# ypw0102/GDR

Measured on AMD Instinct MI355X. Metric: queries/sec on NQ-320k (768-d), higher is better.
Workload: dtype f32; 1 GPU; C2/ragged/prefilter: t5-base encoder 512 q/GPU + Q.D^T top-100, 320000x768 corpus; batch_per_gpu=512, global_batch=512, seq_len=40, corpus_rows=320000, dim=768, k=100, encoder_rows=ragged

## Files before the change

### gdr_amd/_ffi.py

```python
import ctypes as C
import os

_HERE = os.path.dirname(os.path.abspath(__file__))
LIB_PATH = os.environ.get("GDR_HIP_LIB") or os.path.join(_HERE, "libgdr_hip.so")

GDR_OK, GDR_EINVAL, GDR_ENOSPC, GDR_EHIP = 0, -1, -2, -3
ABI_VERSION = 9
RERANK_POSITIONS = 1
RERANK_CHUNKED = 2
SIM_EXHAUSTIVE = 1
SIM_NO_STREAM = 2
EPI_NONE, EPI_RESIDUAL, EPI_RELU, EPI_BIAS, EPI_BIAS_RELU, EPI_BIAS_RESIDUAL, EPI_BIAS_GELU = range(7)
(F32_FORM_TILES, F32_FORM_PERSISTENT, F32_FORM_SMALL, F32_FORM_SMALL_SPLITK, F32_FORM_SPLITK, F32_FORM_STREAMK_256,
 F32_FORM_STREAMK_TAIL) = range(1, 8)
STREAMK_WS_BYTES = 33558528


class GdrError(RuntimeError):
    pass


class GdrT5Dims(C.Structure):
    _fields_ = [("vocab_size", C.c_int32), ("d_model", C.c_int32), ("d_kv", C.c_int32), ("d_ff", C.c_int32),
                ("num_heads", C.c_int32), ("num_layers", C.c_int32), ("rel_buckets", C.c_int32),
# ... 57 lines not shown
SIGNATURES = {
    "gdr_last_error": (C.c_char_p, []),
    "gdr_abi_version": (_i, []),
    "gdr_device_fault_pending": (_i, []),
    "gdr_device_fault_clear": (None, []),
    "gdr_device_fault_inject_for_tests": (None, []),
    "gdr_prof_enable": (_i, [_i]),
    "gdr_prof_collect": (_i, [C.POINTER(C.c_int64), C.POINTER(C.c_double), C.POINTER(C.c_double)]),
    "gdr_linear_f32": (_i, [_vp, _i64, _vp, _i64, _vp, _i64, _i64, _i, _i, _i, _vp, _vp, _i64, _vp]),
    "gdr_linear_bf16": (_i, [_vp, _i64, _vp, _i64, _vp, _i64, _i64, _i, _i, _i, _vp, _vp, _i64, _vp]),
    "gdr_split_row_elems": (_i, [_i, _i]),
    "gdr_split_f32_f16x2": (_i, [_vp, _vp, _i64, _i, _i64, _vp]),
    "gdr_split_f32_bf16x3": (_i, [_vp, _vp, _i64, _i, _i64, _vp]),
    "gdr_linear_split_bf16": (_i, [_vp, _i64, _vp, _i64, _vp, _i64, _i64, _i, _i, _i, _i, _vp, _vp, _i64, _vp]),
    "gdr_linear_bf16_tile_form": (_i, [_i64, _i, _i, _i]),
    "gdr_linear_f32_form": (_i, [_i64, _i, _i, _sz]),
    "gdr_linear_f32_splitk": (_i, [_vp, _i64, _vp, _i64, _vp, _i64, _i64, _i, _i, _i, _vp, _vp, _i64, _vp, _sz, _vp]),
    "gdr_l2_normalize": (_i, [_vp, _vp, _i64, _i, _f, _vp]),
    "gdr_t5_layer_norm": (_i, [_vp, _vp, _vp, _i64, _i, _f, _vp]),
    "gdr_t5_encoder_workspace_bytes": (_sz, [C.POINTER(GdrT5Dims), _i, _i]),
    "gdr_t5_encoder_forward": (_i, [C.POINTER(GdrT5EncoderWeights), _vp, _vp, _i, _i, _vp, _vp, _vp, _sz, _vp]),
    "gdr_t5_encoder_ragged_workspace_bytes": (_sz, [C.POINTER(GdrT5Dims), _i, _i]),
    "gdr_t5_encoder_forward_ragged": (_i, [C.POINTER(GdrT5EncoderWeights), _vp, _vp, _i, _i, _vp, _vp, _i64, _vp, _sz, _vp]),
    "gdr_t5_encoder_forward_ragged_bf16": (_i, [C.POINTER(GdrT5EncoderWeights), _vp, _vp, _i, _i, _vp, _vp, _i64, _vp, _sz, _vp]),
    "gdr_t5_encoder_split_workspace_bytes": (_sz, [C.POINTER(GdrT5Dims), _i, _i]),
    "gdr_t5_encoder_forward_ragged_split": (_i, [C.POINTER(GdrT5EncoderWeights), _vp, _vp, _i, _i, _vp, _vp, _i64, _i, _vp, _sz, _vp]),
    "gdr_t5_encoder_bf16_workspace_bytes": (_sz, [C.POINTER(GdrT5Dims), _i, _i]),
    "gdr_t5_encoder_forward_bf16": (_i, [C.POINTER(GdrT5EncoderWeights), _vp, _vp, _i, _i, _vp, _vp, _vp, _sz, _vp]),
    "gdr_sim_topk_workspace_bytes": (_sz, [_i, _i64, _i, _i, _i]),
    "gdr_sim_topk": (_i, [_vp, _i, _vp, _i64, _i, _i, C.c_int32, _vp, _vp, _vp, _i, _vp, _sz, _vp]),
# ... 104 lines not shown
```

### gdr_amd/csrc/encoder.hip

```cpp
#include <stdlib.h>

#include "layers.h"

namespace gdr {

constexpr size_t ENC_SPLITK_BYTES = (size_t)112 << 20;
static_assert(STREAMK_BYTES <= ENC_SPLITK_BYTES, "stream-K scratch must fit the split-K region");
constexpr bool ENC_LAST_Q_CLS_DEFAULT = true;

static int enc_streamk(char* splitk_region, StreamK* sk, hipStream_t stream) {
  sk->part = reinterpret_cast<float*>(splitk_region);
  sk->flag = reinterpret_cast<int32_t*>(splitk_region + STREAMK_PART_BYTES);
  sk->epoch = 0;
  if (hipMemsetAsync(sk->flag, 0, 512 * sizeof(int32_t), stream) != hipSuccess) {
    set_error("t5_encoder: memset of the stream-K flags failed");
    return GDR_EHIP;
  }
  return GDR_OK;
}

struct EncWs {
  size_t off_h, off_nx, off_qkv, off_ctx, off_ff, off_splitk, off_bf, total;
};

// ... 297 lines not shown
  at.ldq = at.ldk = at.ldv = 3 * inner, at.ldo = inner;
  at.q_bstride = at.k_bstride = at.o_bstride = L;
  at.B = B, at.H = H, at.dk = dk, at.Lq = L, at.Lk = L;
  at.q_pos0 = 0, at.scale = 1.0f;
  at.rel_bias = w->rel_bias, at.bidirectional = 1, at.num_buckets = dm.rel_buckets;
  at.lut = make_bucket_lut(dm.rel_buckets / 2, dm.rel_max_distance);
  at.key_mask = mask, at.mask_bstride = L, at.causal = 0, at.causal_neg_inf = 0;
  at.kv_rows = nullptr, at.kv_group = 1;
  at.seq_off = seq_off, at.seq_len = seq_len;

  const bool pooled_only = out_hidden == nullptr && big;
  static const bool last_q_cls_on = [] {
    const char* e = getenv("GDR_ENC_LAST_Q_CLS");
    return e ? atoi(e) != 0 : ENC_LAST_Q_CLS_DEFAULT;
  }();
  for (int i = 0; i < dm.num_layers; ++i) {
    const GdrT5EncLayer& ly = w->layers[i];
    GDR_CHECK_ARG(ly.ln_attn && ly.wqkv && ly.wo && ly.ln_ff && ly.wi && ly.wo_ff, "t5_encoder_ragged: layer %d null weight", i);
    if (i == 0 && qkv0) {
    } else if (pooled_only && i == dm.num_layers - 1 && last_q_cls_on) {
      if ((rc = launch_rmsnorm_dev(h, ly.ln_attn, nx, rows_dev, M, d, dm.eps, stream))) return rc;
      if ((rc = linear(nx, d, ly.wqkv + (size_t)inner * d, qkv + inner, 3 * inner, 2 * inner, d, GDR_EPI_NONE, nullptr))) return rc;
      if ((rc = launch_gather_rows(nx, seq_off, B, d, nx_cls, stream))) return rc;
      if ((rc = launch_linear_f32(nx_cls, d, ly.wqkv, d, ctx_cls, inner, B, inner, d, GDR_EPI_NONE, nullptr, nullptr, 0, stream)))
        return rc;
      if ((rc = launch_scatter_rows_strided(ctx_cls, seq_off, B, inner, qkv, 3 * inner, stream))) return rc;
    } else {
      if ((rc = launch_rmsnorm_dev(h, ly.ln_attn, nx, rows_dev, M, d, dm.eps, stream))) return rc;
      if ((rc = linear(nx, d, ly.wqkv, qkv, 3 * inner, 3 * inner, d, GDR_EPI_NONE, nullptr))) return rc;
    }
    if ((rc = launch_attention(at, stream))) return rc;
    if (pooled_only && i == dm.num_layers - 1) {
      if ((rc = launch_gather_rows(ctx, seq_off, B, inner, ctx_cls, stream))) return rc;
      if ((rc = launch_gather_rows(h, seq_off, B, d, h_cls, stream))) return rc;
      if ((rc = launch_linear_f32(ctx_cls, inner, ly.wo, inner, h_cls, d, B, d, inner, GDR_EPI_RESIDUAL, nullptr, h_cls, d, stream)))
        return rc;
      if ((rc = launch_rmsnorm(h_cls, ly.ln_ff, nx_cls, B, d, dm.eps, nullptr, 1, stream))) return rc;
      if ((rc = launch_linear_f32(nx_cls, d, ly.wi, d, ff_cls, dm.d_ff, B, dm.d_ff, d, GDR_EPI_RELU, nullptr, nullptr, 0, stream)))
        return rc;
      if ((rc = launch_linear_f32(ff_cls, dm.d_ff, ly.wo_ff, dm.d_ff, h_cls, d, B, d, dm.d_ff, GDR_EPI_RESIDUAL, nullptr, h_cls, d,
                                  stream)))
        return rc;
      return launch_rmsnorm(h_cls, w->final_ln, out_pooled, B, d, dm.eps, nullptr, 1, stream);
    }
    if ((rc = linear(ctx, inner, ly.wo, h, d, d, inner, GDR_EPI_RESIDUAL, h))) return rc;
// ... 193 lines not shown
```

### gdr_amd/csrc/gemm_bf16.hip

```cpp
#include "common.h"

namespace gdr {

typedef float f32x4b __attribute__((ext_vector_type(4)));
typedef __bf16 bf16x8b __attribute__((ext_vector_type(8)));
typedef _Float16 f16x8b __attribute__((ext_vector_type(8)));

struct Bf16GemmArgs {
  const char* A;
  const char* W;
  float* C;
  const float* bias;
  const float* residual;
  int64_t lda, ldw, ldc, ldr;
  int64_t M;
  int64_t Nrows;
  int N, K, tiles_n;
  int has_bias, has_residual, act;
  int out_bf16;
  const int64_t* m_dev;
  int split_k0;
  const float* dot_h;
  int64_t dot_ldh;
  const int32_t* dot_rows;
  const float* dot_e;
  float* dot_out;
  float dot_scale;
  int dot_d;
  SimEpilogue sim;
};

__device__ __forceinline__ float gelu_erf_b(float x) { return 0.5f * x * (1.0f + erff(x * 0.70710678118654752440f)); }

template <int SPLIT>
__device__ __forceinline__ int plane_of(int p, bool is_w) {
  if (SPLIT == 1) return ((is_w ? 0x102010 : 0x120100) >> (4 * p)) & 3;
  return ((is_w ? 0x001 : 0x010) >> (4 * p)) & 3;
}
template <int SPLIT>
__device__ __forceinline__ void ktile_offsets(int kt, int p, int k0, int split_k0, int& off_a, int& off_w) {
  if (SPLIT == 0) {
    off_a = off_w = kt * 128;
    return;
  }
// ... 305 lines not shown
            g.C[m * g.ldc + n + j] = x;
        }
      }
    }
  }
}

#pragma clang diagnostic push
#pragma clang diagnostic ignored "-Winline-asm"
#define GLDS16(gptr_, lds_) \
  asm volatile("s_mov_b32 m0, %0\n\ts_nop 0\n\tglobal_load_lds_dwordx4 %1, off" ::"s"(lds_), "v"(gptr_) : "memory", "m0")

constexpr int HALF_BYTES = 128 * 128;
constexpr int OFF_A_LO = 0, OFF_A_HI = HALF_BYTES, OFF_B_LO = 2 * HALF_BYTES, OFF_B_HI = 3 * HALF_BYTES, BUF_BYTES = 4 * HALF_BYTES;

template <int BN, int SPLIT = 0>
__global__ __launch_bounds__(512, 1) void gemm_nt_bf16_tile256_kernel(const Bf16GemmArgs g) {
  static_assert(BN == 256 || BN == 192, "tile width");
  constexpr int WCOLS = BN / 4;
  constexpr int NBH = BN == 256 ? 2 : 1;
  constexpr int NB = 2 + NBH;
  constexpr int HI_ROWS = 16 * NBH;
  extern __shared__ __attribute__((aligned(1024))) char smem256[];
  unsigned bid = blockIdx.x;
  const int64_t Mv = g.m_dev ? *g.m_dev : g.M;
  const int tiles_n = (g.N + BN - 1) / BN;
  {
    unsigned nblk = gridDim.x;
    if (g.m_dev) {
      const int64_t live = ((Mv + 255) / 256) * (int64_t)tiles_n;
      if (live < (int64_t)nblk) {
        if ((int64_t)bid >= live) return;
        nblk = (unsigned)live;
      }
    }
    const unsigned q_ = nblk >> 3, r_ = nblk & 7u, xcd_ = bid & 7u, j_ = bid >> 3;
    bid = (xcd_ < r_ ? xcd_ * (q_ + 1) : r_ * (q_ + 1) + (xcd_ - r_) * q_) + j_;
  }
  const int64_t m0 = (int64_t)(bid / (unsigned)tiles_n) * 256;
  if (m0 >= Mv) return;
  const int n0 = (int)(bid % (unsigned)tiles_n) * BN;
  const int tid = threadIdx.x, wave = tid >> 6, lane = tid & 63;
  const int wr = wave >> 2, wc = wave & 3, r16 = lane & 15, q4 = lane >> 4;
  const unsigned lds0 = __builtin_amdgcn_readfirstlane((unsigned)(uintptr_t)(__attribute__((address_space(3))) char*)(smem256));
  const int srow = lane >> 3, schunk = lane & 7;
  const char* a_src[2][2];
  const char* b_lo_src[2];
  const char* b_hi_src[NBH];
#pragma unroll
  for (int h = 0; h < 2; ++h)
#pragma unroll
    for (int i = 0; i < 2; ++i) {
      const int lr = (wave * 2 + i) * 8 + srow;
      const int chunk = schunk ^ ((lr >> 1) & 7);
      int64_t ra = m0 + (lr >> 6) * 128 + h * 64 + (lr & 63);
      ra = ra < Mv ? ra : Mv - 1;
      a_src[h][i] = g.A + (ra * g.lda) * 2 + chunk * 16;
    }
#pragma unroll
  for (int i = 0; i < 2; ++i) {
    const int lr = (wave * 2 + i) * 8 + srow;
    const int chunk = schunk ^ ((lr >> 1) & 7);
    int rb = n0 + (lr >> 5) * WCOLS + (lr & 31);
    rb = rb < g.N ? rb : g.N - 1;
    b_lo_src[i] = g.W + ((int64_t)rb * g.ldw) * 2 + chunk * 16;
  }
#pragma unroll
  for (int i = 0; i < NBH; ++i) {
    const int lr = NBH == 2 ? (wave * 2 + i) * 8 + srow : wave * 8 + srow;
    const int chunk = schunk ^ ((lr >> 1) & 7);
    int rb = n0 + (lr / HI_ROWS) * WCOLS + 32 + (lr % HI_ROWS);
    rb = rb < g.N ? rb : g.N - 1;
    b_hi_src[i] = g.W + ((int64_t)rb * g.ldw) * 2 + chunk * 16;
  }
  const unsigned st_dst = lds0 + (unsigned)__builtin_amdgcn_readfirstlane(wave) * 2048;
  const unsigned st_dst1 = lds0 + (unsigned)__builtin_amdgcn_readfirstlane(wave) * 1024;
#define STAGE(src_, half_off_, buf_, koff_)                                                 \
  {                                                                                         \
    GLDS16(src_[0] + (koff_), st_dst + (buf_)*BUF_BYTES + (half_off_));                     \
    GLDS16(src_[1] + (koff_), st_dst + (buf_)*BUF_BYTES + (half_off_) + 1024);              \
  }
#define STAGE_BHI(buf_, koff_)                                                              \
  {                                                                                         \
    if (NBH == 2) STAGE(b_hi_src, OFF_B_HI, buf_, koff_)                                    \
    else GLDS16(b_hi_src[0] + (koff_), st_dst1 + (buf_)*BUF_BYTES + OFF_B_HI);              \
  }
  const int sw = (r16 >> 1) & 7;
  const int c0 = (q4 ^ sw) << 4;
// ... 127 lines not shown
    STAGE(a_src[0], OFF_A_LO, 1, a_o3)
    BAR()
    asm volatile("s_waitcnt lgkmcnt(0)" ::: "memory");
    __builtin_amdgcn_sched_barrier(0);
    MFMA_Q(1, 2, NBH, fbh)
    BAR()
    STAGE_BHI(1, w_o3)
    WAIT_3HALVES()
    BAR()
    MFMA_Q(1, 0, 2, fbl)
    BAR()
    a_o1 = a_o3;
  }
  asm volatile("s_waitcnt vmcnt(0)" ::: "memory");
  if (wr == 0) BAR()
#pragma unroll
  for (int mi = 0; mi < 8; ++mi) {
    const int64_t m = m0 + wr * 128 + mi * 16 + r16;
    if (m >= Mv) continue;
#pragma unroll
    for (int ni = 0; ni < NB; ++ni) {
      const int n = n0 + wc * WCOLS + ni * 16 + 4 * q4;
      if (n >= g.N) continue;
      float v[4] = {acc[mi][ni][0], acc[mi][ni][1], acc[mi][ni][2], acc[mi][ni][3]};
      if (g.has_bias) {
        const float4 b = *reinterpret_cast<const float4*>(g.bias + n);
        v[0] += b.x, v[1] += b.y, v[2] += b.z, v[3] += b.w;
      }
      if (g.has_residual) {
        const float4 r = *reinterpret_cast<const float4*>(g.residual + m * g.ldr + n);
// ... 136 lines not shown
  g.lda = lda, g.ldw = ldw, g.M = M, g.N = N, g.Nrows = N, g.K = K;
  g.tiles_n = N / 128;
  g.m_dev = m_dev;
  g.dot_h = h, g.dot_ldh = ldh, g.dot_rows = rows_map, g.dot_e = E, g.dot_out = partial, g.dot_scale = scale, g.dot_d = dot_d;
  int64_t blocks = ((M + 127) / 128) * g.tiles_n;
  if (blocks <= 0) return 0;
  if (blocks > 0x7fffffffLL) {
    set_error("linear_bf16(head dot): grid too large");
    return GDR_EINVAL;
  }
  hipLaunchKernelGGL((gemm_nt_bf16_glds_kernel<3, 128>), dim3((unsigned)blocks), dim3(256), 0, stream, g);
  GDR_CHECK_LAUNCH("gemm_nt_bf16_glds_kernel(head dot)");
  return 0;
}

int launch_sim_bf16_glds(const void* D, int64_t N, const void* Q, int B, int d, const SimEpilogue& ep, int64_t n_doc_tiles,
                         hipStream_t stream) {
  if (d % 64 != 0 || ((uintptr_t)D & 15) || ((uintptr_t)Q & 15)) return 1;
  Bf16GemmArgs g{};
  g.A = static_cast<const char*>(Q), g.W = static_cast<const char*>(D);
  g.lda = d, g.ldw = d, g.M = B, g.Nrows = N, g.N = 0, g.K = d;
  g.tiles_n = (B + 127) / 128;
  g.sim = ep;
  const int64_t blocks = n_doc_tiles * g.tiles_n;
  if (blocks <= 0) return 0;
  if (blocks > 0x7fffffffLL) {
    set_error("sim_bf16: grid too large");
    return GDR_EINVAL;
  }
  if (ep.mode == 1)
    hipLaunchKernelGGL(gemm_nt_bf16_glds_kernel<1>, dim3((unsigned)blocks), dim3(256), 0, stream, g);
  else
    hipLaunchKernelGGL(gemm_nt_bf16_glds_kernel<2>, dim3((unsigned)blocks), dim3(256), 0, stream, g);
  GDR_CHECK_LAUNCH("gemm_nt_bf16_glds_kernel(sim)");
  return 0;
}

}

extern "C" int gdr_linear_bf16_tile_form(int64_t M, int N, int K, int epilogue) {
  const int has_residual = epilogue == GDR_EPI_RESIDUAL || epilogue == GDR_EPI_BIAS_RESIDUAL;
  return gdr::linear_bf16_tile_form(M, N, K, has_residual, 0);
}

namespace gdr {
__global__ __launch_bounds__(256) void split_f32_bf16x3_kernel(const float* __restrict__ in, int64_t ld_in, __bf16* __restrict__ out,
                                                              int64_t ld_out, int64_t rows, int K, const int64_t* __restrict__ rows_dev,
                                                              int form) {
  const int k4 = K >> 2;
  const int64_t i = (int64_t)blockIdx.x * 256 + threadIdx.x;
  const int64_t r = i / k4;
  const int c = (int)(i - r * k4) * 4;
  if (r >= (rows_dev ? *rows_dev : rows)) return;
// ... 53 lines not shown
```

### gdr_amd/csrc/gemm_small.hip

```cpp
#include <stdlib.h>

#include "common.h"

namespace gdr {

typedef float f32x16m __attribute__((ext_vector_type(16)));

constexpr int SB = 64, SBK = 32, SLD = SBK + 4;

struct SmallGemmArgs {
  const float* A;
  const float* W;
  float* C;
  const float* bias;
  const float* residual;
  int64_t lda, ldw, ldc, ldr;
  int64_t M;
  int N, K, tiles_n, tiles_m;
  int has_bias, has_residual, act;
  int ksplit, kchunk;
  const int64_t* m_dev;
  const int32_t* live;
};

// ... 97 lines not shown
#undef S_STORE
#undef S_COMPUTE
  if (g.ksplit > 1) {
    float* slab = g.C + ((int64_t)tile * g.ksplit + split) * (SB * SB);
#pragma unroll
    for (int r = 0; r < 16; ++r) slab[(wm * 32 + (r & 3) + 8 * (r >> 2) + 4 * h) * SB + wn * 32 + l31] = acc[r];
    return;
  }
  const int n = n0 + wn * 32 + l31;
  if (n >= g.N) return;
  const float bia = g.has_bias ? g.bias[n] : 0.f;
#pragma unroll
  for (int r = 0; r < 16; ++r) {
    const int64_t m = m0 + wm * 32 + (r & 3) + 8 * (r >> 2) + 4 * h;
    if (m >= Mrows) continue;
    float v = acc[r] + bia;
    if (g.has_residual) v += g.residual[m * g.ldr + n];
    if (g.act == 1) v = fmaxf(v, 0.f);
    if (g.act == 2) v = gelu_erf_s(v);
    g.C[m * g.ldc + n] = v;
  }
}

__global__ __launch_bounds__(256) void splitk_reduce_small_kernel(const float* __restrict__ partial, int S, int tiles_n,
                                                                  int64_t M, int N, float* __restrict__ C, int64_t ldc,
                                                                  const float* __restrict__ bias,
                                                                  const float* __restrict__ residual, int64_t ldr,
                                                                  int act, const int64_t* __restrict__ m_dev,
                                                                  const int32_t* __restrict__ live) {
  if (live && *live == 0) return;
// ... 139 lines not shown
  SmallGemmArgs g{};
  g.A = A, g.W = W, g.bias = bias, g.residual = residual;
  g.lda = lda, g.ldw = ldw, g.ldc = ldc, g.ldr = ldr, g.M = M, g.N = N, g.K = K, g.tiles_n = tiles_n;
  g.ksplit = S, g.kchunk = chunk_steps * SBK;
  g.m_dev = m_dev, g.live = live;
  g.tiles_m = (int)tiles_m;
  const double flops = 2.0 * (double)M * (double)N * (double)K;
  if (ne && (S == 1 || N % 4 != 0 || N > 1024 || act > 1)) return 2;
  if (slabs) {
    if (has_bias || has_residual || act || ne) return 1;
    slabs->part = nullptr, slabs->S = 1, slabs->tiles_n = tiles_n;
  }
  if (S == 1) {
    g.C = C, g.has_bias = has_bias, g.has_residual = has_residual, g.act = act;
    ProfScope prof(PROF_LINEAR, flops, stream);
    hipLaunchKernelGGL(gemm_nt_f32_small_kernel, dim3((unsigned)tiles), dim3(256), 0, stream, g);
    GDR_CHECK_LAUNCH("gemm_nt_f32_small_kernel");
    return 0;
  }
  g.C = ws;
  {
    ProfScope prof(PROF_LINEAR, flops, stream);
    hipLaunchKernelGGL(gemm_nt_f32_small_kernel, dim3((unsigned)(tiles * S)), dim3(256), 0, stream, g);
  }
  GDR_CHECK_LAUNCH("gemm_nt_f32_small_kernel(split)");
  if (slabs) {
    slabs->part = ws, slabs->S = S, slabs->tiles_n = tiles_n;
    return 0;
  }
  ProfScope prof_r(PROF_REDUCE, 0.0, stream);
// ... 16 lines not shown
```

### gdr_amd/csrc/layers.h

```cpp
#pragma once
#include "common.h"

namespace gdr {

struct BucketLut {
  uint8_t v[128];
};
BucketLut make_bucket_lut(int nb, int max_distance);

struct AttnArgs {
  const float* q;
  const float* k;
  const float* v;
  float* out;
  void* out_bf16;
  int64_t ldq, ldk, ldv, ldo;
  int64_t q_bstride, k_bstride, o_bstride;
  int B, H, dk, Lq, Lk;
  int q_pos0;
  float scale;
  const float* rel_bias;
  int bidirectional, num_buckets;
  BucketLut lut;
  const int64_t* key_mask;
  int64_t mask_bstride;
  int causal;
  int causal_neg_inf;
  const int32_t* kv_rows;
  int kv_group;
  int q_same_pos;
  const int32_t* seq_off;
  const int32_t* seq_len;
  int qkv_bf16;
  const int64_t* b_count_dev;
  const float* q_part;
  int q_S, q_tiles_n;
  const int32_t* live;
};
int launch_attention(const AttnArgs& a, hipStream_t stream);
int launch_attention_long(const AttnArgs& a, hipStream_t stream);

int launch_embed(const float* table, const int64_t* ids, int64_t rows, int d, int vocab, float* out,
                 hipStream_t stream);
int launch_pack_plan(const int64_t* mask, int B, int L, int32_t* seq_len, int32_t* seq_off, int32_t* row_src,
                     int64_t* rows_total, hipStream_t stream);
int launch_embed_packed(const float* table, const int64_t* ids, const int32_t* row_src, const int64_t* rows_dev,
                        int64_t max_rows, int d, int vocab, float* out, hipStream_t stream);
int launch_embed_packed2(const float* table, const float* table2, const int64_t* ids, const int32_t* row_src,
                         const int64_t* rows_dev, int64_t max_rows, int d, int e, int vocab, float* out, float* out2,
                         hipStream_t stream);
int launch_gather_rows(const float* src, const int32_t* idx, int n, int d, float* dst, hipStream_t stream);
int launch_scatter_rows_strided(const float* src, const int32_t* idx, int n, int d, float* dst, int64_t ldd, hipStream_t stream);
// ... 21 lines not shown
```

### gdr_amd/csrc/layers.hip

```cpp
#include <math.h>

#include <stdlib.h>

#include "layers.h"

namespace gdr {

BucketLut make_bucket_lut(int nb, int max_distance) {
  BucketLut l;
  const int max_exact = nb / 2;
  for (int n = 0; n < 128; ++n) {
    int b;
    if (n < max_exact) {
      b = n;
    } else {
      const float v = logf((float)n / (float)max_exact) / (float)log((double)max_distance / max_exact) *
                      (float)(nb - max_exact);
      b = max_exact + (int)v;
      if (b > nb - 1) b = nb - 1;
    }
    l.v[n] = (uint8_t)b;
  }
  return l;
}
// ... 683 lines not shown
  constexpr int DK = 64, DS = DK + 4, LP = 16 * NT, NTHR = 64 * NT;
  const int Lr = a.Lk;
  float* Ks = smem;
  float* Vs = Ks + Lr * DS;
  float* RelB = Vs + Lr * DS;
  float* Mk = RelB + 2 * LP;
  const int b = blockIdx.x / a.H, h = blockIdx.x % a.H;
  const int L = a.seq_len ? a.seq_len[b] : a.Lk, tid = threadIdx.x;
  const int64_t qrow0 = a.seq_off ? a.seq_off[b] : (int64_t)b * a.q_bstride;
  const int64_t krow0 = a.seq_off ? a.seq_off[b] : (int64_t)b * a.k_bstride;
  const int64_t orow0 = a.seq_off ? a.seq_off[b] : (int64_t)b * a.o_bstride;
  float4 qv[DK / 16];
  {
    const int wq = tid >> 6, lq = tid & 63;
    const int64_t qr = qrow0 + min(16 * wq + (lq & 15), L - 1);
    if (16 * wq < L) {
      if (a.qkv_bf16) {
        const __bf16* q16 = reinterpret_cast<const __bf16*>(a.q) + qr * a.ldq + h * DK + 4 * (lq >> 4);
#pragma unroll
        for (int jj = 0; jj < DK / 16; ++jj) {
          const uint2 u = *reinterpret_cast<const uint2*>(q16 + 16 * jj);
          qv[jj] = make_float4(__uint_as_float(u.x << 16) * a.scale, __uint_as_float(u.x & 0xffff0000u) * a.scale,
                               __uint_as_float(u.y << 16) * a.scale, __uint_as_float(u.y & 0xffff0000u) * a.scale);
        }
      } else {
        const float* q32 = a.q + qr * a.ldq + h * DK + 4 * (lq >> 4);
#pragma unroll
        for (int jj = 0; jj < DK / 16; ++jj) qv[jj] = *reinterpret_cast<const float4*>(q32 + 16 * jj);
      }
    }
  }
// ... 71 lines not shown
        *reinterpret_cast<float4*>(Vs + r * DS + 4 * c) = vst[it];
      }
    }
    if (tid < 2 * LP) RelB[tid] = rb_val;
  }
  if (a.qkv_bf16 && tid < 2 * LP) RelB[tid] = rb_bucket >= 0 ? a.rel_bias[(rb_base[0] + rb_lut[0]) * a.H + h] : 0.f;
  if (tid < LP) Mk[tid] = tid < L ? ((mk_mine && mk_raw == 0) ? (a.causal_neg_inf ? -INFINITY : -1e9f) : 0.f) : -INFINITY;
  __syncthreads();
  if (!a.qkv_bf16) {
#pragma unroll
    for (int jj = 0; jj < DK / 16; ++jj) qv[jj].x *= a.scale, qv[jj].y *= a.scale, qv[jj].z *= a.scale, qv[jj].w *= a.scale;
  }

  const int w = tid >> 6, lane = tid & 63, c16 = lane & 15, q4 = lane >> 4;
  if (16 * w >= L) return;
  const int nt_live = (L + 15) >> 4;
  f32x4_t st[NT];
#pragma unroll
  for (int t = 0; t < NT; ++t) st[t] = (f32x4_t){0.f, 0.f, 0.f, 0.f};
#pragma unroll
  for (int jj = 0; jj < DK / 16; ++jj) {
#pragma unroll
    for (int t = 0; t < NT; ++t) {
      if (t >= nt_live) continue;
      const float4 kv = *reinterpret_cast<const float4*>(Ks + min(16 * t + c16, L - 1) * DS + 4 * q4 + 16 * jj);
      st[t] = __builtin_amdgcn_mfma_f32_16x16x4f32(kv.x, qv[jj].x, st[t], 0, 0, 0);
      st[t] = __builtin_amdgcn_mfma_f32_16x16x4f32(kv.y, qv[jj].y, st[t], 0, 0, 0);
      st[t] = __builtin_amdgcn_mfma_f32_16x16x4f32(kv.z, qv[jj].z, st[t], 0, 0, 0);
      st[t] = __builtin_amdgcn_mfma_f32_16x16x4f32(kv.w, qv[jj].w, st[t], 0, 0, 0);
    }
// ... 817 lines not shown
```

### gdr_amd/csrc/sim_topk.hip

```cpp
#include <stdlib.h>

#include "common.h"

namespace gdr {

constexpr int TILE = 128;
constexpr int SEL_THREADS = 256;

struct SimPlan {
  int64_t tiles_m;
  int stride;
  int64_t n_sample_tiles;
  int64_t n_slots;
  int64_t cap;
  size_t off_val, off_idx, off_cnt, off_thr, off_part, total;
};

static SimPlan make_plan(int B, int64_t N, int k, bool exhaustive, double survivors = 1.0) {
  SimPlan p{};
  p.tiles_m = (N + TILE - 1) / TILE;
  double target = sqrt((double)k * (double)N);
  if (target < k) target = k;
  int64_t ts = (int64_t)((target + TILE - 1) / TILE);
  if (ts < 1) ts = 1;
// ... 686 lines not shown
  float best = 0.f;
  for (int64_t r = (int64_t)blockIdx.x * 4 + (threadIdx.x >> 6); r < N; r += (int64_t)gridDim.x * 4) {
    const float* row = D + r * d;
    float ss = 0.f;
    for (int c = lane * 4; c < d; c += 256) {
      const float4 v = *reinterpret_cast<const float4*>(row + c);
      ss = fmaf(v.x, v.x, fmaf(v.y, v.y, fmaf(v.z, v.z, fmaf(v.w, v.w, ss))));
    }
#pragma unroll
    for (int off = 32; off > 0; off >>= 1) ss += __shfl_xor(ss, off);
    best = fmaxf(best, ss);
  }
  if (lane == 0) atomicMax(out, __float_as_uint(best));
}

template <int RC>
__global__ __launch_bounds__(1024) void prefilter_tail_kernel(const float* __restrict__ cand_val, const int32_t* __restrict__ cand_idx,
                                                              const int32_t* __restrict__ cand_cnt, int64_t cap, int k, int cap2,
                                                              int cap2p, const float* __restrict__ eps2, const float* __restrict__ Q,
                                                              const float* __restrict__ D, int d, int32_t idx_offset,
                                                              float* __restrict__ out_val, int32_t* __restrict__ out_idx,
                                                              int32_t* __restrict__ status) {
  __shared__ int hist[256];
  __shared__ int scan[256];
  __shared__ int res[2];
  __shared__ uint32_t red[32];
  __shared__ int n_sh;
  extern __shared__ __attribute__((aligned(16))) unsigned long long pkeys[];
  const int q = blockIdx.x, tid = threadIdx.x, lane = tid & 63, wave = tid >> 6;
  const int c_all = cand_cnt[(int64_t)q * CNT_STRIDE], count = c_all < (int)cap ? c_all : (int)cap;
  const float* v = cand_val + (int64_t)q * cap;
// ... 78 lines not shown
      }
    }
  }
  __syncthreads();
  const int n_all = n_sh, n2 = n_all < cap2 ? n_all : cap2;
  if (tid == 0 && status) status[q] = (c_all > (int)cap || n_all > cap2) ? 1 : 0;
  {
    constexpr int MAXP = 4;
    float4 qr[MAXP];
#pragma unroll
    for (int t = 0; t < MAXP; ++t) {
      const int col = lane * 4 + 256 * t;
      qr[t] = col < d ? *reinterpret_cast<const float4*>(Q + (int64_t)q * d + col) : make_float4(0.f, 0.f, 0.f, 0.f);
    }
    float* vals = reinterpret_cast<float*>(pkeys);
    for (int i0 = wave * 2; i0 < n2; i0 += 32) {
      const int i1 = i0 + 1 < n2 ? i0 + 1 : i0;
      const int64_t r0 = ids[i0], r1 = ids[i1];
      float4 a0[MAXP], a1[MAXP];
#pragma unroll
      for (int t = 0; t < MAXP; ++t) {
        const int col = lane * 4 + 256 * t;
        a0[t] = col < d ? *reinterpret_cast<const float4*>(D + r0 * d + col) : make_float4(0.f, 0.f, 0.f, 0.f);
        a1[t] = col < d ? *reinterpret_cast<const float4*>(D + r1 * d + col) : make_float4(0.f, 0.f, 0.f, 0.f);
      }
      float s0 = 0.f, s1 = 0.f;
#pragma unroll
      for (int t = 0; t < MAXP; ++t) {
        s0 = fmaf(qr[t].x, a0[t].x, s0), s0 = fmaf(qr[t].y, a0[t].y, s0), s0 = fmaf(qr[t].z, a0[t].z, s0), s0 = fmaf(qr[t].w, a0[t].w, s0);
        s1 = fmaf(qr[t].x, a1[t].x, s1), s1 = fmaf(qr[t].y, a1[t].y, s1), s1 = fmaf(qr[t].z, a1[t].z, s1), s1 = fmaf(qr[t].w, a1[t].w, s1);
      }
// ... 136 lines not shown
  hipLaunchKernelGGL(sim_qprep_kernel, dim3(B), dim3(256), 0, stream, Q, d, dnorm_max, Q16, eps2);
  GDR_CHECK_LAUNCH("sim_qprep_kernel");
  const bool stream_mode = sim_stream_supported(B, d, true);
  int rc = stream_mode ? launch_sim_stream(D_bf16, N, Q16, B, d, ep, true, stream) : launch_sim_gemm(D_bf16, N, Q16, B, d, ep, true, stream);
  if (rc) return rc;
  hipLaunchKernelGGL(sim_threshold_kernel, dim3(B), dim3(1024), 0, stream, ep.cand_val, p.cap, (int)p.n_slots, k, thr, ep.cand_cnt,
                     (const float*)eps2);
  GDR_CHECK_LAUNCH("sim_threshold_kernel");
  if (p.stride > 1) {
    ep.mode = 2;
    rc = stream_mode ? launch_sim_stream(D_bf16, N, Q16, B, d, ep, true, stream) : launch_sim_gemm(D_bf16, N, Q16, B, d, ep, true, stream);
    if (rc) return rc;
  }
  int cap2p = 1024;
  while (cap2p < pp.cap2) cap2p <<= 1;
  if (int rc__ = ensure_dyn_lds(reinterpret_cast<const void*>(prefilter_tail_kernel<16>), cap2p * 8, "sim_topk_prefilter")) return rc__;
  hipLaunchKernelGGL(prefilter_tail_kernel<16>, dim3(B), dim3(1024), (size_t)cap2p * 8, stream, (const float*)ep.cand_val,
                     (const int32_t*)ep.cand_idx, (const int32_t*)ep.cand_cnt, p.cap, k, pp.cap2, cap2p, (const float*)eps2, Q, D, d,
                     idx_offset, out_val, out_idx, status);
  GDR_CHECK_LAUNCH("prefilter_tail_kernel");
  return GDR_OK;
}

extern "C" int gdr_topk_merge(const float* vals, const int32_t* idx, int G, int B, int k, float* out_val,
                              int32_t* out_idx, void* stream_) {
  using namespace gdr;
  hipStream_t stream = static_cast<hipStream_t>(stream_);
  if (B == 0) return GDR_OK;
  GDR_CHECK_ARG(vals && idx && out_val && out_idx, "topk_merge: null pointer");
  GDR_CHECK_ARG(G > 0 && B > 0 && k >= 1 && k <= 1024, "topk_merge: bad shape G=%d B=%d k=%d", G, B, k);
  const int kpad = next_pow2(k);
  hipLaunchKernelGGL(topk_select_kernel<true>, dim3(B), dim3(SEL_THREADS), kpad * sizeof(unsigned long long), stream,
// ... 55 lines not shown
```

### include/gdr_hip.h

```cpp
#ifndef GDR_HIP_H
#define GDR_HIP_H

#include <stddef.h>
#include <stdint.h>

#ifdef __cplusplus
extern "C" {
#endif

#define GDR_OK 0
#define GDR_EINVAL (-1)
#define GDR_ENOSPC (-2)
#define GDR_EHIP (-3)

const char* gdr_last_error(void);
int gdr_abi_version(void);
int64_t gdr_launch_count(void);

int gdr_prof_enable(int max_events);
int gdr_prof_collect(int64_t* launches, double* total_ms, double* total_work);
void gdr_prof_gate(int on);

enum {
  GDR_EPI_NONE = 0,
// ... 16 lines not shown
#define GDR_F32_FORM_SMALL 3
#define GDR_F32_FORM_SMALL_SPLITK 4
#define GDR_F32_FORM_SPLITK 5
#define GDR_F32_FORM_STREAMK_256 6
#define GDR_F32_FORM_STREAMK_TAIL 7
int gdr_linear_f32_form(int64_t M, int N, int K, size_t workspace_bytes);

int gdr_linear_bf16(const void* A, int64_t lda, const void* W, int64_t ldw, float* C, int64_t ldc, int64_t M, int N,
                    int K, int epilogue, const float* bias, const float* residual, int64_t ldr, void* stream);
int gdr_split_row_elems(int K, int terms);
int gdr_split_f32_bf16x3(const float* in, void* out_planes, int64_t rows, int K, int64_t ld_out, void* stream);
int gdr_split_f32_f16x2(const float* in, void* out_planes, int64_t rows, int K, int64_t ld_out, void* stream);
int gdr_linear_split_bf16(const void* A3, int64_t lda, const void* W3, int64_t ldw, float* C, int64_t ldc, int64_t M, int N, int K,
                          int terms, int epilogue, const float* bias, const float* residual, int64_t ldr, void* stream);
int gdr_linear_bf16_tile_form(int64_t M, int N, int K, int epilogue);

int gdr_t5_layer_norm(const float* x, const float* w, float* y, int64_t rows, int d, float eps, void* stream);

int gdr_l2_normalize(const float* x, float* y, int64_t rows, int d, float eps, void* stream);

typedef struct {
  int32_t vocab_size, d_model, d_kv, d_ff, num_heads, num_layers;
  int32_t rel_buckets, rel_max_distance;
  float eps;
} GdrT5Dims;

typedef struct {
  const float* ln_attn;
  const float* wqkv;
  const float* wo;
// ... 243 lines not shown
```

Baseline: 31150 queries/s.

## Add 256-wide bf16 similarity tile, fine small GEMM, CLS-only attention, wider prefilter tail

New measurement: 31100 queries/s. Within noise of the previous version (-0.2%).

```diff
diff --git a/gdr_amd/_ffi.py b/gdr_amd/_ffi.py
--- a/gdr_amd/_ffi.py
+++ b/gdr_amd/_ffi.py
@@ -95,6 +95,7 @@
     "gdr_split_f32_bf16x3": (_i, [_vp, _vp, _i64, _i, _i64, _vp]),
     "gdr_linear_split_bf16": (_i, [_vp, _i64, _vp, _i64, _vp, _i64, _i64, _i, _i, _i, _i, _vp, _vp, _i64, _vp]),
     "gdr_linear_bf16_tile_form": (_i, [_i64, _i, _i, _i]),
+    "gdr_sim_bf16_tile_form": (_i, [_i, _i]),
     "gdr_linear_f32_form": (_i, [_i64, _i, _i, _sz]),
     "gdr_linear_f32_splitk": (_i, [_vp, _i64, _vp, _i64, _vp, _i64, _i64, _i, _i, _i, _vp, _vp, _i64, _vp, _sz, _vp]),
     "gdr_l2_normalize": (_i, [_vp, _vp, _i64, _i, _f, _vp]),
diff --git a/gdr_amd/csrc/encoder.hip b/gdr_amd/csrc/encoder.hip
--- a/gdr_amd/csrc/encoder.hip
+++ b/gdr_amd/csrc/encoder.hip
@@ -335,6 +335,10 @@
     const char* e = getenv("GDR_ENC_LAST_Q_CLS");
     return e ? atoi(e) != 0 : ENC_LAST_Q_CLS_DEFAULT;
   }();
+  static const bool last_attn_cls_on = [] {
+    const char* e = getenv("GDR_ENC_LAST_ATTN_CLS");
+    return !(e && e[0] == '0');
+  }();
   for (int i = 0; i < dm.num_layers; ++i) {
     const GdrT5EncLayer& ly = w->layers[i];
     GDR_CHECK_ARG(ly.ln_attn && ly.wqkv && ly.wo && ly.ln_ff && ly.wi && ly.wo_ff, "t5_encoder_ragged: layer %d null weight", i);
@@ -350,6 +354,7 @@
       if ((rc = launch_rmsnorm_dev(h, ly.ln_attn, nx, rows_dev, M, d, dm.eps, stream))) return rc;
       if ((rc = linear(nx, d, ly.wqkv, qkv, 3 * inner, 3 * inner, d, GDR_EPI_NONE, nullptr))) return rc;
     }
+    if (pooled_only && i == dm.num_layers - 1 && last_attn_cls_on) at.q_tiles = 1;
     if ((rc = launch_attention(at, stream))) return rc;
     if (pooled_only && i == dm.num_layers - 1) {
       if ((rc = launch_gather_rows(ctx, seq_off, B, inner, ctx_cls, stream))) return rc;
diff --git a/gdr_amd/csrc/gemm_bf16.hip b/gdr_amd/csrc/gemm_bf16.hip
--- a/gdr_amd/csrc/gemm_bf16.hip
+++ b/gdr_amd/csrc/gemm_bf16.hip
@@ -1,3 +1,5 @@
+#include <stdlib.h>
+
 #include "common.h"
 
 namespace gdr {
@@ -28,6 +30,7 @@
   float dot_scale;
   int dot_d;
   SimEpilogue sim;
+  int64_t sim_tiles;
 };
 
 __device__ __forceinline__ float gelu_erf_b(float x) { return 0.5f * x * (1.0f + erff(x * 0.70710678118654752440f)); }
@@ -363,9 +366,10 @@
 constexpr int HALF_BYTES = 128 * 128;
 constexpr int OFF_A_LO = 0, OFF_A_HI = HALF_BYTES, OFF_B_LO = 2 * HALF_BYTES, OFF_B_HI = 3 * HALF_BYTES, BUF_BYTES = 4 * HALF_BYTES;
 
-template <int BN, int SPLIT = 0>
+template <int BN, int SPLIT = 0, int EPI = 0>
 __global__ __launch_bounds__(512, 1) void gemm_nt_bf16_tile256_kernel(const Bf16GemmArgs g) {
   static_assert(BN == 256 || BN == 192, "tile width");
+  static_assert(EPI == 0 || (BN == 256 && SPLIT == 0), "the similarity forms: plain bf16 rows, 256 docs");
   constexpr int WCOLS = BN / 4;
   constexpr int NBH = BN == 256 ? 2 : 1;
   constexpr int NB = 2 + NBH;
@@ -373,7 +377,7 @@
   extern __shared__ __attribute__((aligned(1024))) char smem256[];
   unsigned bid = blockIdx.x;
   const int64_t Mv = g.m_dev ? *g.m_dev : g.M;
-  const int tiles_n = (g.N + BN - 1) / BN;
+  const int tiles_n = EPI ? g.tiles_n : (g.N + BN - 1) / BN;
   {
     unsigned nblk = gridDim.x;
     if (g.m_dev) {
@@ -386,9 +390,17 @@
     const unsigned q_ = nblk >> 3, r_ = nblk & 7u, xcd_ = bid & 7u, j_ = bid >> 3;
     bid = (xcd_ < r_ ? xcd_ * (q_ + 1) : r_ * (q_ + 1) + (xcd_ - r_) * q_) + j_;
   }
-  const int64_t m0 = (int64_t)(bid / (unsigned)tiles_n) * 256;
+  const int64_t m0 = (int64_t)(EPI ? bid % (unsigned)tiles_n : bid / (unsigned)tiles_n) * 256;
   if (m0 >= Mv) return;
-  const int n0 = (int)(bid % (unsigned)tiles_n) * BN;
+  const int n0 = EPI ? 0 : (int)(bid % (unsigned)tiles_n) * BN;
+  const int64_t sim_pair = EPI ? (int64_t)(bid / (unsigned)tiles_n) * 2 : 0;
+  auto sim_col0 = [&](int c) -> int64_t {
+    const int64_t f = sim_pair + (c >> 1);
+    if (f >= g.sim_tiles) return g.Nrows;
+    const int64_t s1 = g.sim.tile_stride - 1;
+    const int64_t dt = EPI == 1 ? f * g.sim.tile_stride : (f / s1) * g.sim.tile_stride + 1 + (f % s1);
+    return dt * 128 + (c & 1) * 64;
+  };
   const int tid = threadIdx.x, wave = tid >> 6, lane = tid & 63;
   const int wr = wave >> 2, wc = wave & 3, r16 = lane & 15, q4 = lane >> 4;
   const unsigned lds0 = __builtin_amdgcn_readfirstlane((unsigned)(uintptr_t)(__attribute__((address_space(3))) char*)(smem256));
@@ -410,17 +422,19 @@
   for (int i = 0; i < 2; ++i) {
     const int lr = (wave * 2 + i) * 8 + srow;
     const int chunk = schunk ^ ((lr >> 1) & 7);
-    int rb = n0 + (lr >> 5) * WCOLS + (lr & 31);
-    rb = rb < g.N ? rb : g.N - 1;
-    b_lo_src[i] = g.W + ((int64_t)rb * g.ldw) * 2 + chunk * 16;
+    int64_t rb = EPI ? sim_col0(lr >> 5) + (lr & 31) : (int64_t)(n0 + (lr >> 5) * WCOLS + (lr & 31));
+    const int64_t rb_end = EPI ? g.Nrows : (int64_t)g.N;
+    rb = rb < rb_end ? rb : rb_end - 1;
+    b_lo_src[i] = g.W + (rb * g.ldw) * 2 + chunk * 16;
   }
 #pragma unroll
   for (int i = 0; i < NBH; ++i) {
     const int lr = NBH == 2 ? (wave * 2 + i) * 8 + srow : wave * 8 + srow;
     const int chunk = schunk ^ ((lr >> 1) & 7);
-    int rb = n0 + (lr / HI_ROWS) * WCOLS + 32 + (lr % HI_ROWS);
-    rb = rb < g.N ? rb : g.N - 1;
-    b_hi_src[i] = g.W + ((int64_t)rb * g.ldw) * 2 + chunk * 16;
+    int64_t rb = EPI ? sim_col0(lr / HI_ROWS) + 32 + (lr % HI_ROWS) : (int64_t)(n0 + (lr / HI_ROWS) * WCOLS + 32 + (lr % HI_ROWS));
+    const int64_t rb_end = EPI ? g.Nrows : (int64_t)g.N;
+    rb = rb < rb_end ? rb : rb_end - 1;
+    b_hi_src[i] = g.W + (rb * g.ldw) * 2 + chunk * 16;
   }
   const unsigned st_dst = lds0 + (unsigned)__builtin_amdgcn_readfirstlane(wave) * 2048;
   const unsigned st_dst1 = lds0 + (unsigned)__builtin_amdgcn_readfirstlane(wave) * 1024;
@@ -578,6 +592,71 @@
   }
   asm volatile("s_waitcnt vmcnt(0)" ::: "memory");
   if (wr == 0) BAR()
+  if constexpr (EPI != 0) {
+    const int64_t nb = sim_col0(wc);
+    if (sim_pair + (wc >> 1) >= g.sim_tiles) return;
+    if (EPI == 1) {
+      const int64_t slot_base = (sim_pair + (wc >> 1)) * 128 + (wc & 1) * 64;
+#pragma unroll
+      for (int mi = 0; mi < 8; ++mi) {
+        const int64_t q = m0 + wr * 128 + mi * 16 + r16;
+        if (q >= Mv) continue;
+        float* cv = g.sim.cand_val + q * g.sim.cap + slot_base;
+        int32_t* ci = g.sim.cand_idx + q * g.sim.cap + slot_base;
+#pragma unroll
+        for (int ni = 0; ni < 4; ++ni) {
+          const int off = ni * 16 + 4 * q4;
+          const int64_t n = nb + off;
+          float4 v;
+          int4 id;
+          v.x = n + 0 < g.Nrows ? acc[mi][ni][0] : -INFINITY, v.y = n + 1 < g.Nrows ? acc[mi][ni][1] : -INFINITY;
+          v.z = n + 2 < g.Nrows ? acc[mi][ni][2] : -INFINITY, v.w = n + 3 < g.Nrows ? acc[mi][ni][3] : -INFINITY;
+          id.x = n + 0 < g.Nrows ? (int)n : -1, id.y = n + 1 < g.Nrows ? (int)n + 1 : -1;
+          id.z = n + 2 < g.Nrows ? (int)n + 2 : -1, id.w = n + 3 < g.Nrows ? (int)n + 3 : -1;
+          *reinterpret_cast<float4*>(cv + off) = v;
+          *reinterpret_cast<int4*>(ci + off) = id;
+        }
+      }
+      return;
+    }
+#pragma unroll
+    for (int mi = 0; mi < 8; ++mi) {
+      const int64_t q = m0 + wr * 128 + mi * 16 + r16;
+      const bool q_ok = q < Mv;
+      const float thr = q_ok ? g.sim.thr[q] : INFINITY;
+      unsigned keep = 0u;
+#pragma unroll
+      for (int ni = 0; ni < 4; ++ni)
+#pragma unroll
+        for (int r = 0; r < 4; ++r) {
+          const int64_t n = nb + ni * 16 + 4 * q4 + r;
+          keep |= (q_ok && acc[mi][ni][r] >= thr && n < g.Nrows) ? (1u << (4 * ni + r)) : 0u;
+        }
+      const int mine = __popc(keep);
+      const int c0 = __shfl(mine, r16), c1 = __shfl(mine, r16 + 16), c2 = __shfl(mine, r16 + 32), c3 = __shfl(mine, r16 + 48);
+      const int total = c0 + c1 + c2 + c3;
+      int base = 0;
+      if (q4 == 0 && total > 0) base = atomicAdd(g.sim.cand_cnt + (int64_t)q * CNT_STRIDE, total);
+      base = __shfl(base, r16);
+      int pos = base + (q4 > 0 ? c0 : 0) + (q4 > 1 ? c1 : 0) + (q4 > 2 ? c2 : 0);
+      if (mine) {
+        float* cv = g.sim.cand_val + q * g.sim.cap;
+        int32_t* ci = g.sim.cand_idx + q * g.sim.cap;
+#pragma unroll
+        for (int ni = 0; ni < 4; ++ni)
+#pragma unroll
+          for (int r = 0; r < 4; ++r)
+            if (keep >> (4 * ni + r) & 1u) {
+              if (pos < g.sim.cap) {
+                cv[pos] = acc[mi][ni][r];
+                ci[pos] = (int)(nb + ni * 16 + 4 * q4 + r);
+              }
+              ++pos;
+            }
+      }
+    }
+    return;
+  }
 #pragma unroll
   for (int mi = 0; mi < 8; ++mi) {
     const int64_t m = m0 + wr * 128 + mi * 16 + r16;
@@ -744,6 +823,15 @@
   return 0;
 }
 
+int sim_bf16_tile_form(int B, int d) {
+  static const bool tile256 = [] {
+    const char* e = getenv("GDR_SIM_TILE256");
+    return !(e && e[0] == '0');
+  }();
+  if (B <= 0 || d <= 0 || d % 64 != 0) return 0;
+  return tile256 && B >= 129 && d % 128 == 0 ? 256 : 128;
+}
+
 int launch_sim_bf16_glds(const void* D, int64_t N, const void* Q, int B, int d, const SimEpilogue& ep, int64_t n_doc_tiles,
                          hipStream_t stream) {
   if (d % 64 != 0 || ((uintptr_t)D & 15) || ((uintptr_t)Q & 15)) return 1;
@@ -758,6 +846,20 @@
     set_error("sim_bf16: grid too large");
     return GDR_EINVAL;
   }
+  if (sim_bf16_tile_form(B, d) == 256) {
+    g.tiles_n = (B + 255) / 256;
+    g.sim_tiles = n_doc_tiles;
+    const int64_t b256 = ((n_doc_tiles + 1) / 2) * g.tiles_n;
+    if (ep.mode == 1) {
+      if (int rc__ = ensure_dyn_lds(reinterpret_cast<const void*>(gemm_nt_bf16_tile256_kernel<256, 0, 1>), 2 * BUF_BYTES, "sim_bf16")) return rc__;
+      hipLaunchKernelGGL((gemm_nt_bf16_tile256_kernel<256, 0, 1>), dim3((unsigned)b256), dim3(512), 2 * BUF_BYTES, stream, g);
+    } else {
+      if (int rc__ = ensure_dyn_lds(reinterpret_cast<const void*>(gemm_nt_bf16_tile256_kernel<256, 0, 2>), 2 * BUF_BYTES, "sim_bf16")) return rc__;
+      hipLaunchKernelGGL((gemm_nt_bf16_tile256_kernel<256, 0, 2>), dim3((unsigned)b256), dim3(512), 2 * BUF_BYTES, stream, g);
+    }
+    GDR_CHECK_LAUNCH("gemm_nt_bf16_tile256_kernel(sim)");
+    return 0;
+  }
   if (ep.mode == 1)
     hipLaunchKernelGGL(gemm_nt_bf16_glds_kernel<1>, dim3((unsigned)blocks), dim3(256), 0, stream, g);
   else
@@ -767,6 +869,8 @@
 }
 
 }
+
+extern "C" int gdr_sim_bf16_tile_form(int B, int d) { return gdr::sim_bf16_tile_form(B, d); }
 
 extern "C" int gdr_linear_bf16_tile_form(int64_t M, int N, int K, int epilogue) {
   const int has_residual = epilogue == GDR_EPI_RESIDUAL || epilogue == GDR_EPI_BIAS_RESIDUAL;
diff --git a/gdr_amd/csrc/gemm_small.hip b/gdr_amd/csrc/gemm_small.hip
--- a/gdr_amd/csrc/gemm_small.hip
+++ b/gdr_amd/csrc/gemm_small.hip
@@ -135,6 +135,102 @@
   for (int r = 0; r < 16; ++r) {
     const int64_t m = m0 + wm * 32 + (r & 3) + 8 * (r >> 2) + 4 * h;
     if (m >= Mrows) continue;
+    float v = acc[r] + bia;
+    if (g.has_residual) v += g.residual[m * g.ldr + n];
+    if (g.act == 1) v = fmaxf(v, 0.f);
+    if (g.act == 2) v = gelu_erf_s(v);
+    g.C[m * g.ldc + n] = v;
+  }
+}
+
+typedef float f32x4m __attribute__((ext_vector_type(4)));
+constexpr int FB = 32, FBK = 64, FLD = FBK + 4;
+
+__global__ __launch_bounds__(256, 4) void gemm_nt_f32_small_fine_kernel(const SmallGemmArgs g) {
+  __shared__ __attribute__((aligned(16))) float smem[2 * 2 * FB * FLD];
+  float* const As = smem;
+  float* const Bs = smem + 2 * FB * FLD;
+  unsigned bid = blockIdx.x;
+  {
+    const unsigned nblk = gridDim.x, q = nblk >> 3, r = nblk & 7u, xcd = bid & 7u, j = bid >> 3;
+    bid = (xcd < r ? xcd * (q + 1) : r * (q + 1) + (xcd - r) * q) + j;
+  }
+  const unsigned tiles_m = (unsigned)g.tiles_m;
+  const unsigned tile = (bid % tiles_m) * (unsigned)g.tiles_n + bid / tiles_m;
+  const int64_t m0 = (int64_t)(tile / (unsigned)g.tiles_n) * FB;
+  const int n0 = (int)(tile % (unsigned)g.tiles_n) * FB;
+  const int tid = threadIdx.x;
+  const int lrow = tid >> 3, lcol = 16 * ((tid & 7) >> 1) + 4 * (tid & 1);
+  int64_t ra = m0 + lrow;
+  ra = ra < g.M ? ra : g.M - 1;
+  int rw = n0 + lrow;
+  rw = rw < g.N ? rw : g.N - 1;
+  const float* const a_src = g.A + ra * g.lda + lcol;
+  const float* const w_src = g.W + (int64_t)rw * g.ldw + lcol;
+  const int st_off = lrow * FLD + lcol;
+  const int wave = tid >> 6, lane = tid & 63, wm = wave >> 1, wn = wave & 1, r16 = lane & 15, g4 = lane >> 4;
+  const int a_rd = (wm * 16 + r16) * FLD + 4 * g4;
+  const int b_rd = (wn * 16 + r16) * FLD + 4 * g4;
+  const int nk = g.K / FBK;
+
+  f32x4m acc = {0.f, 0.f, 0.f, 0.f};
+  float4 pa0, pa1, pb0, pb1, qa0, qa1, qb0, qb1;
+#define F_LOAD(R, kt_)                                                                       \
+  {                                                                                          \
+    const int t_ = (kt_) < nk ? (kt_) : nk - 1;    \
+    R##a0 = *reinterpret_cast<const float4*>(a_src + t_ * FBK);                              \
+    R##a1 = *reinterpret_cast<const float4*>(a_src + t_ * FBK + 8);                          \
+    R##b0 = *reinterpret_cast<const float4*>(w_src + t_ * FBK);                              \
+    R##b1 = *reinterpret_cast<const float4*>(w_src + t_ * FBK + 8);                          \
+  }
+#define F_STORE(R, buf_)                                                                     \
+  {                                                                                          \
+    float* as_ = As + (buf_)*FB * FLD + st_off;                                              \
+    float* bs_ = Bs + (buf_)*FB * FLD + st_off;                                              \
+    *reinterpret_cast<float4*>(as_) = make_float4(R##a0.x, R##a0.z, R##a1.x, R##a1.z);       \
+    *reinterpret_cast<float4*>(as_ + 8) = make_float4(R##a0.y, R##a0.w, R##a1.y, R##a1.w);   \
+    *reinterpret_cast<float4*>(bs_) = make_float4(R##b0.x, R##b0.z, R##b1.x, R##b1.z);       \
+    *reinterpret_cast<float4*>(bs_ + 8) = make_float4(R##b0.y, R##b0.w, R##b1.y, R##b1.w);   \
+  }
+#define F_COMPUTE(buf_)                                                                      \
+  {                                                                                          \
+    const float* a = As + (buf_)*FB * FLD + a_rd;                                            \
+    const float* b = Bs + (buf_)*FB * FLD + b_rd;                                            \
+    _Pragma("unroll") for (int jj = 0; jj < 4; ++jj) {                                       \
+      const float4 av = *reinterpret_cast<const float4*>(a + 16 * jj);                       \
+      const float4 bv = *reinterpret_cast<const float4*>(b + 16 * jj);                       \
+      acc = __builtin_amdgcn_mfma_f32_16x16x4f32(av.x, bv.x, acc, 0, 0, 0);                  \
+      acc = __builtin_amdgcn_mfma_f32_16x16x4f32(av.y, bv.y, acc, 0, 0, 0);                  \
+      acc = __builtin_amdgcn_mfma_f32_16x16x4f32(av.z, bv.z, acc, 0, 0, 0);                  \
+      acc = __builtin_amdgcn_mfma_f32_16x16x4f32(av.w, bv.w, acc, 0, 0, 0);                  \
+    }                                                                                        \
+  }
+  F_LOAD(p, 0)
+  F_STORE(p, 0)
+  F_LOAD(p, 1)
+  F_LOAD(q, 2)
+  __syncthreads();
+  for (int kt = 0; kt < nk; kt += 2) {
+    F_COMPUTE(0)
+    F_STORE(p, 1)
+    F_LOAD(p, kt + 3)
+    __syncthreads();
+    if (kt + 1 >= nk) break;
+    F_COMPUTE(1)
+    F_STORE(q, 0)
+    F_LOAD(q, kt + 4)
+    __syncthreads();
+  }
+#undef F_LOAD
+#undef F_STORE
+#undef F_COMPUTE
+  const int n = n0 + wn * 16 + r16;
+  if (n >= g.N) return;
+  const float bia = g.has_bias ? g.bias[n] : 0.f;
+#pragma unroll
+  for (int r = 0; r < 4; ++r) {
+    const int64_t m = m0 + wm * 16 + 4 * g4 + r;
+    if (m >= g.M) continue;
     float v = acc[r] + bia;
     if (g.has_residual) v += g.residual[m * g.ldr + n];
     if (g.act == 1) v = fmaxf(v, 0.f);
@@ -304,6 +400,16 @@
   if (S == 1) {
     g.C = C, g.has_bias = has_bias, g.has_residual = has_residual, g.act = act;
     ProfScope prof(PROF_LINEAR, flops, stream);
+    static const bool fine = [] {
+      const char* e = getenv("GDR_SMALL_FINE");
+      return !(e && e[0] == '0');
+    }();
+    if (fine && tiles < 128 && K % FBK == 0 && !m_dev && !live) {
+      g.tiles_m = (int)((M + FB - 1) / FB), g.tiles_n = (N + FB - 1) / FB;
+      hipLaunchKernelGGL(gemm_nt_f32_small_fine_kernel, dim3((unsigned)(g.tiles_m * g.tiles_n)), dim3(256), 0, stream, g);
+      GDR_CHECK_LAUNCH("gemm_nt_f32_small_fine_kernel");
+      return 0;
+    }
     hipLaunchKernelGGL(gemm_nt_f32_small_kernel, dim3((unsigned)tiles), dim3(256), 0, stream, g);
     GDR_CHECK_LAUNCH("gemm_nt_f32_small_kernel");
     return 0;
diff --git a/gdr_amd/csrc/layers.h b/gdr_amd/csrc/layers.h
--- a/gdr_amd/csrc/layers.h
+++ b/gdr_amd/csrc/layers.h
@@ -36,6 +36,7 @@
   const float* q_part;
   int q_S, q_tiles_n;
   const int32_t* live;
+  int q_tiles;
 };
 int launch_attention(const AttnArgs& a, hipStream_t stream);
 int launch_attention_long(const AttnArgs& a, hipStream_t stream);
diff --git a/gdr_amd/csrc/layers.hip b/gdr_amd/csrc/layers.hip
--- a/gdr_amd/csrc/layers.hip
+++ b/gdr_amd/csrc/layers.hip
@@ -721,7 +721,7 @@
   {
     const int wq = tid >> 6, lq = tid & 63;
     const int64_t qr = qrow0 + min(16 * wq + (lq & 15), L - 1);
-    if (16 * wq < L) {
+    if (16 * wq < L && (a.q_tiles == 0 || wq < a.q_tiles)) {
       if (a.qkv_bf16) {
         const __bf16* q16 = reinterpret_cast<const __bf16*>(a.q) + qr * a.ldq + h * DK + 4 * (lq >> 4);
 #pragma unroll
@@ -823,6 +823,7 @@
 
   const int w = tid >> 6, lane = tid & 63, c16 = lane & 15, q4 = lane >> 4;
   if (16 * w >= L) return;
+  if (a.q_tiles && w >= a.q_tiles) return;
   const int nt_live = (L + 15) >> 4;
   f32x4_t st[NT];
 #pragma unroll
diff --git a/gdr_amd/csrc/sim_topk.hip b/gdr_amd/csrc/sim_topk.hip
--- a/gdr_amd/csrc/sim_topk.hip
+++ b/gdr_amd/csrc/sim_topk.hip
@@ -724,7 +724,7 @@
   if (lane == 0) atomicMax(out, __float_as_uint(best));
 }
 
-template <int RC>
+template <int RC, bool WIDE>
 __global__ __launch_bounds__(1024) void prefilter_tail_kernel(const float* __restrict__ cand_val, const int32_t* __restrict__ cand_idx,
                                                               const int32_t* __restrict__ cand_cnt, int64_t cap, int k, int cap2,
                                                               int cap2p, const float* __restrict__ eps2, const float* __restrict__ Q,
@@ -833,7 +833,36 @@
       qr[t] = col < d ? *reinterpret_cast<const float4*>(Q + (int64_t)q * d + col) : make_float4(0.f, 0.f, 0.f, 0.f);
     }
     float* vals = reinterpret_cast<float*>(pkeys);
-    for (int i0 = wave * 2; i0 < n2; i0 += 32) {
+    for (int i0 = wave * 4; WIDE && i0 < n2; i0 += 64) {
+      constexpr int NR = 4;
+      float4 a[NR][MAXP];
+#pragma unroll
+      for (int u = 0; u < NR; ++u) {
+        const int64_t r = ids[i0 + u < n2 ? i0 + u : n2 - 1];
+#pragma unroll
+        for (int t = 0; t < MAXP; ++t) {
+          const int col = lane * 4 + 256 * t;
+          a[u][t] = col < d ? *reinterpret_cast<const float4*>(D + r * d + col) : make_float4(0.f, 0.f, 0.f, 0.f);
+        }
+      }
+      float sc[NR];
+#pragma unroll
+      for (int u = 0; u < NR; ++u) {
+        float s0 = 0.f;
+#pragma unroll
+        for (int t = 0; t < MAXP; ++t)
+          s0 = fmaf(qr[t].x, a[u][t].x, s0), s0 = fmaf(qr[t].y, a[u][t].y, s0), s0 = fmaf(qr[t].z, a[u][t].z, s0), s0 = fmaf(qr[t].w, a[u][t].w, s0);
+        sc[u] = s0;
+      }
+#pragma unroll
+      for (int u = 0; u < NR; ++u) sc[u] = wave_sum(sc[u]);
+      if (lane == 0) {
+#pragma unroll
+        for (int u = 0; u < NR; ++u)
+          if (i0 + u < n2) vals[i0 + u] = sc[u];
+      }
+    }
+    for (int i0 = wave * 2; !WIDE && i0 < n2; i0 += 32) {
       const int i1 = i0 + 1 < n2 ? i0 + 1 : i0;
       const int64_t r0 = ids[i0], r1 = ids[i1];
       float4 a0[MAXP], a1[MAXP];
@@ -1000,8 +1029,13 @@
   }
   int cap2p = 1024;
   while (cap2p < pp.cap2) cap2p <<= 1;
-  if (int rc__ = ensure_dyn_lds(reinterpret_cast<const void*>(prefilter_tail_kernel<16>), cap2p * 8, "sim_topk_prefilter")) return rc__;
-  hipLaunchKernelGGL(prefilter_tail_kernel<16>, dim3(B), dim3(1024), (size_t)cap2p * 8, stream, (const float*)ep.cand_val,
+  static const bool tail_wide = [] {
+    const char* e = getenv("GDR_PREFILTER_TAIL");
+    return !(e && e[0] == '0');
+  }();
+  const auto tail = tail_wide ? prefilter_tail_kernel<16, true> : prefilter_tail_kernel<16, false>;
+  if (int rc__ = ensure_dyn_lds(reinterpret_cast<const void*>(tail), cap2p * 8, "sim_topk_prefilter")) return rc__;
+  hipLaunchKernelGGL(tail, dim3(B), dim3(1024), (size_t)cap2p * 8, stream, (const float*)ep.cand_val,
                      (const int32_t*)ep.cand_idx, (const int32_t*)ep.cand_cnt, p.cap, k, pp.cap2, cap2p, (const float*)eps2, Q, D, d,
                      idx_offset, out_val, out_idx, status);
   GDR_CHECK_LAUNCH("prefilter_tail_kernel");
diff --git a/include/gdr_hip.h b/include/gdr_hip.h
--- a/include/gdr_hip.h
+++ b/include/gdr_hip.h
@@ -54,6 +54,7 @@
 int gdr_linear_split_bf16(const void* A3, int64_t lda, const void* W3, int64_t ldw, float* C, int64_t ldc, int64_t M, int N, int K,
                           int terms, int epilogue, const float* bias, const float* residual, int64_t ldr, void* stream);
 int gdr_linear_bf16_tile_form(int64_t M, int N, int K, int epilogue);
+int gdr_sim_bf16_tile_form(int B, int d);
 
 int gdr_t5_layer_norm(const float* x, const float* w, float* y, int64_t rows, int d, float eps, void* stream);
 
```
